# UnofficialJuliaMirrorSnapshots/TrajectoryOptimization.jl-c79d492b-0548-5874-b488-5a62c1d9d0ca

Hardware: AMD Instinct MI355X
Metric: iLQR iterations/sec (batched trajectories), quadrotor n=13 m=4 N=101 (higher is better)
Workload: dtype f64

## Files before the change

### trajectoryoptimization.jl-c79d492b-0548-5874-b488-5a62c1d9d0ca_amd/csrc/tog_bwd_team.hpp

```cpp
#pragma once
#include <type_traits>

namespace tog {

#define TEAM_FENCE() asm volatile("" ::: "memory")

constexpr int PX = 20;

template <class M>
struct TeamCfg {
  static constexpr int n = M::n, m = M::m, L = n + m;
  static constexpr int TEAM = (n + 1 <= 8) ? 8 : 16;
  static constexpr int TPW = WAVE / TEAM;
  static constexpr int cmax(int a, int b) { return a > b ? a : b; }
  static constexpr int PU = 2 * m;
  static constexpr int BUS =
      cmax(cmax(n * L, 3 * n * m), cmax(cmax(32 + n * m + n, n * n + n), cmax(m * m + n * m, n + PX + 2)));
  static constexpr int R2 = cmax(L * n, n * n + n);
  static constexpr int BUSP = cmax(BUS, n * L + R2);
  static constexpr int R2S = cmax(3 * m * m, m * m + 1);
  static constexpr int BUSPS = cmax(BUS, n * L + R2S);
  static constexpr int RQ = cmax(2 * n, n + PX);
};

// ... 13 lines not shown
__host__ __device__ inline int bwd_team_stride(int , int sqrt) {
  using C = TeamCfg<M>;
  int s = sqrt ? C::BUSPS : C::BUSP;
  s += sreg_size<M>(sqrt != 0);
  s += (34 - s % 32) % 32;
  return s;
}
inline size_t bwd_team_shmem(int stride, int tpw, int , int N) {
  return sizeof(double) * (size_t)stride * tpw + sizeof(int) * 2 * (size_t)N;
}

template <class M>
__host__ __device__ constexpr int ne_of() {
  return M::n + M::m + M::m * M::m + M::n * M::n;
}
constexpr int QPK = 4;
template <bool SQRT, bool AL>
__device__ __forceinline__ bool knot_dense(int k, int N, int cnt, int nx) {
  return k == N - 1 || (AL && (SQRT ? nx > 0 : cnt > 0));
}
template <class M>
__host__ __device__ inline int expand_team_stride(int pmax) {
  int s = 48 + pmax * 8 + pmax + M::n + M::m;
  return s + (s & 1);
}

constexpr int TEAM_MAX_ROWS = 128;
constexpr int TEAM_MAX_KNOTS = 1024;
inline bool team_rows_fit(const int* knot_off, const int* knot_cnt, const ConRow* rows, int N, int n, int m,
                          int nrows) {
  if (n + 1 > 16 || m > n || nrows > TEAM_MAX_ROWS || N > TEAM_MAX_KNOTS) return false;
  for (int k = 0; k < N; k++) {
    int nx = 0, nu = 0;
    if (knot_cnt[k] > PCAP) return false;
    for (int r = 0; r < knot_cnt[k]; r++) {
      const int t = rows[knot_off[k] + r].type;
      if (t == ROW_USER_INEQ || t == ROW_USER_EQ) return false;
      if (t == ROW_UMAX || t == ROW_UMIN) nu++;
      else nx++;
    }
    if (nx > PX || nu > 2 * m) return false;
  }
  return true;
}

template <class M, bool PT>
__device__ __forceinline__ void team_rows(const DevProblem* P, const DevBuffers& Bf, long long b, int k, int N, int pmax, int p,
                                          const ConRow* cr, const double* x, const double* u, RowInfo* rows,
                                          int* xr, int* ur, int& nx, int& nu, int team, int tl, int TEAM) {
  constexpr int n = M::n;
  const double* lam = Bf.lam + ((size_t)b * N + k) * pmax;
  const double* mu = Bf.mu + ((size_t)b * N + k) * pmax;
  const unsigned long long tmask = (TEAM >= 64 ? ~0ull : ((1ull << TEAM) - 1ull)) << (team * TEAM);
  const unsigned long long below = tmask & ((1ull << threadIdx.x) - 1ull);
  int cx = 0, cu = 0;
  for (int base = 0; base < p; base += TEAM) {
    const int r = base + tl;
    bool isx = false, isu = false;
    if (r < p) {
      const ConRow row = traj_row<PT>(P, b, cr[r]);
      const double c = row_value<false>(row, x, u);
      const double l = lam[r];
      const bool a = row_inequality<false>(row) ? ((c >= 0.0) || (l > 0.0)) : true;
      RowInfo ri;
      ri.w = a ? mu[r] : 0.0;
      ri.ws = a ? sqrt(mu[r]) : 0.0;
      ri.g = ri.w * c + l;
      ri.nnz = row_grad<false>(row, x, n, ri.idx, ri.v);
      rows[r] = ri;
      isu = (row.type == ROW_UMAX || row.type == ROW_UMIN);
      isx = !isu;
    }
    const unsigned long long bx = __ballot(isx) & tmask, bu = __ballot(isu) & tmask;
    if (isx) xr[cx + __popcll(bx & below)] = r;
    if (isu) ur[cu + __popcll(bu & below)] = r;
    cx += __popcll(bx);
    cu += __popcll(bu);
  }
  nx = cx;
  nu = cu;
}

__device__ __forceinline__ double row_at(const RowInfo& r, int col) {
  double v = 0.0;
  for (int z = 0; z < r.nnz; z++)
    if (r.idx[z] == col) v = r.v[z];
  return v;
}

template <class T>
__device__ __forceinline__ T opaque(T v) {
  asm volatile("" : "+v"(v));
  return v;
}

template <int L>
__device__ __forceinline__ double row_bcast(double v) {
  return __builtin_amdgcn_update_dpp(__builtin_nondeterministic_value(v), v, 0x150 + L, 0xF, 0xF, true);
}

template <int L>
__device__ __forceinline__ double quad_bcast(double v) {
  const long long x = __builtin_bit_cast(long long, v);
  const int lo = __builtin_amdgcn_update_dpp(__builtin_nondeterministic_value(0), (int)(x & 0xffffffffll), L * 0x55,
                                             0xF, 0xF, true);
  const int hi = __builtin_amdgcn_update_dpp(__builtin_nondeterministic_value(0), (int)(x >> 32), L * 0x55, 0xF, 0xF,
                                             true);
// ... 374 lines not shown
          team_qr<m + PU, m, m, TEAM, true>(a, m + PU, tl, bus);
        else
          team_qr<m + PU, m, m, TEAM>(a, m + nu, tl, bus);
#pragma unroll
        for (int i = 0; i < m; i++) Quuc[i] = (i <= tl) ? a[i] : 0.0;
      }
    }
    {
      double tx = 0.0;
      for (int z = 0; z < nx; z++) {
        const RowInfo& ri = rows[xr[z]];
        const double v = colx ? row_at(ri, c) : 0.0;
        if (v != 0.0) tx = fma(v, ri.g, tx);
      }
      Qxs += tx;
      if (!TERM) {
        double tu[m];
#pragma unroll
        for (int i = 0; i < m; i++) tu[i] = 0.0;
        for (int z = 0; z < nu; z++) {
          const RowInfo& ri = rows[ur[z]];
          const int id = ri.idx[0];
#pragma unroll
          for (int i = 0; i < m; i++)
            if (id == n + i) tu[i] = fma(ri.v[0], ri.g, tu[i]);
        }
#pragma unroll
        for (int i = 0; i < m; i++) Qu[i] += tu[i];
      }
    }
  }
  double* e = Bf.E + ((size_t)b * N + k) * NE;
  if (colx) e[tl] = Qxs;
  if (!TERM) {
    if (colu) {
      double qu = Qu[0];
#pragma unroll
      for (int i = 1; i < m; i++)
        if (tl == i) qu = Qu[i];
      e[n + tl] = qu;
#pragma unroll
      for (int i = 0; i < m; i++) e[n + m + i + m * tl] = Quuc[i];
    }
  }
  int nxk = 0;
  if (AL && SQRT) nxk = P->knot_nx[k];
  if (colx && knot_dense<SQRT, AL>(k, N, p, nxk)) {
#pragma unroll
    for (int i = 0; i < n; i++) e[n + m + m * m + i + n * tl] = Qxc[i];
  }
}

template <class M, int SQRTI, int ALI>
__global__ void __launch_bounds__(64) k_expand_team(const DevProblem* P, DevBuffers Bf, int mode) {
  using Cfg = TeamCfg<M>;
  extern __shared__ double expand_lds[];
  const int team = threadIdx.x / Cfg::TEAM, tl = threadIdx.x % Cfg::TEAM;
  const int N = P->N;
  const long long idx = (long long)blockIdx.x * Cfg::TPW + team;
  const long long slot = (mode == 2) ? idx : idx / N;
  const int k = (mode == 2) ? N - 1 : (int)(idx - slot * N);
  const long long b = traj_of_slot(Bf, slot, P->B);
  if (b < 0) return;
  if (!Bf.st[b].active || Bf.st[b].ls_pend) return;
  if (mode == 1 && k < N - 1 && !((ALI & 1) && P->knot_nx[k] > 0)) return;
  double* tlds = expand_lds + (size_t)team * expand_team_stride<M>(P->pmax);
  if (k == N - 1)
    team_expand<M, SQRTI != 0, (ALI & 1) != 0, true, (ALI & 2) != 0>(P, Bf, b, k, tlds, tl, team);
  else
    team_expand<M, SQRTI != 0, (ALI & 1) != 0, false, (ALI & 2) != 0>(P, Bf, b, k, tlds, tl, team);
}

template <class M, bool AL, bool PT>
__device__ __forceinline__ void quad_expand(const DevProblem* P, const DevBuffers& Bf, long long b, int k, int tl) {
  using Cfg = TeamCfg<M>;
  constexpr int n = M::n, m = M::m, PU = Cfg::PU, NE = ne_of<M>(), TQ = 4;
  static_assert(m <= TQ, "quad_expand: at most 4 controls");
  const int N = P->N, pmax = P->pmax;
  const double dt = P->dt;
  const bool colu = tl < m;
  const int cu = colu ? tl : 0;
  const double* xg = Bf.X + ((size_t)b * N + k) * n;
  const double* ug = Bf.U + ((size_t)b * (N - 1) + k) * m;
  constexpr int NXL = (n + TQ - 1) / TQ;
  double Qxs[NXL], Quuc[m], Qu[m];
  const int diag_mode = P->diag_cost;
  const CostView C_ = cost_at<n, m, PT>(P, k, b);
  if (diag_mode == 2) {
#pragma unroll
    for (int j = 0; j < NXL; j++) {
      const int cc = tl + TQ * j < n ? tl + TQ * j : 0;
      Qxs[j] = ((fma(C_.Q[cc + n * cc], xg[cc], 0.0) + C_.q[cc]) + 0.0) * dt;
    }
#pragma unroll
    for (int i = 0; i < m; i++) Qu[i] = ((fma(C_.R[i + m * i], ug[i], 0.0) + C_.r[i]) + 0.0) * dt;
    const double rd = C_.cR[cu + m * cu];
#pragma unroll
    for (int i = 0; i < m; i++) Quuc[i] = (i == cu) ? rd : 0.0;
  } else {
#pragma unroll
    for (int j = 0; j < NXL; j++) {
      const int cc = tl + TQ * j < n ? tl + TQ * j : 0;
      double a = 0.0, bq = 0.0;
      if (diag_mode) {
        a = fma(C_.Q[cc + n * cc], xg[cc], 0.0);
      } else {
#pragma unroll
        for (int jj = 0; jj < n; jj++) a = fma(C_.Q[cc + n * jj], xg[jj], a);
#pragma unroll
        for (int jj = 0; jj < m; jj++) bq = fma(C_.H[jj + m * cc], ug[jj], bq);
      }
      Qxs[j] = ((a + C_.q[cc]) + bq) * dt;
    }
#pragma unroll
    for (int i = 0; i < m; i++) {
      double a2 = 0.0, b2 = 0.0;
      if (diag_mode) {
        a2 = fma(C_.R[i + m * i], ug[i], 0.0);
      } else {
#pragma unroll
        for (int j = 0; j < m; j++) a2 = fma(C_.R[i + m * j], ug[j], a2);
#pragma unroll
        for (int j = 0; j < n; j++) b2 = fma(C_.H[i + m * j], xg[j], b2);
// ... 39 lines not shown
      return __builtin_amdgcn_update_dpp(__builtin_nondeterministic_value(0), rid[i / TQ], (i % TQ) * 0x55, 0xF, 0xF,
                                         true);
    };
    {
      double a[m + PU];
#pragma unroll
      for (int i = 0; i < m; i++) a[i] = Quuc[i];
      static_for<0, PU>([&](auto ic) {
        constexpr int i = decltype(ic)::value;
        const double ws = quad_bcast<i % TQ>(rws[i / TQ]), v = quad_bcast<i % TQ>(rv[i / TQ]);
        const int id = idx_of(ic);
        a[m + i] = (i < nu) ? ws * ((id == n + cu) ? v : 0.0) : 0.0;
      });
      team_qr<m + PU, m, m, TQ, true>(a, m + PU, tl, nullptr);
#pragma unroll
      for (int i = 0; i < m; i++) Quuc[i] = (i <= tl) ? a[i] : 0.0;
    }
    double tu[m];
#pragma unroll
    for (int i = 0; i < m; i++) tu[i] = 0.0;
    static_for<0, PU>([&](auto zc) {
      constexpr int z = decltype(zc)::value;
      const double v = quad_bcast<z % TQ>(rv[z / TQ]), g = quad_bcast<z % TQ>(rg[z / TQ]);
      const int id = idx_of(zc);
      if (z < nu) {
#pragma unroll
        for (int i = 0; i < m; i++)
          if (id == n + i) tu[i] = fma(v, g, tu[i]);
      }
    });
#pragma unroll
    for (int i = 0; i < m; i++) Qu[i] += tu[i];
    {
#pragma unroll
      for (int j = 0; j < NXL; j++) Qxs[j] += 0.0;
    }
  }
  double* e = Bf.E + ((size_t)b * N + k) * NE;
#pragma unroll
  for (int j = 0; j < NXL; j++)
    if (tl + TQ * j < n) e[tl + TQ * j] = Qxs[j];
  if (colu) {
    double qu = Qu[0];
#pragma unroll
    for (int i = 1; i < m; i++)
      if (tl == i) qu = Qu[i];
    e[n + tl] = qu;
#pragma unroll
    for (int i = 0; i < m; i++) e[n + m + i + m * tl] = Quuc[i];
  }
}

template <class M, int ALI>
__global__ void __launch_bounds__(64) __attribute__((amdgpu_waves_per_eu(5))) k_expand_u(const DevProblem* P, DevBuffers Bf) {
  const int team = threadIdx.x / 4, tl = threadIdx.x % 4;
  const int N = P->N;
  const long long idx = (long long)blockIdx.x * 16 + team;
  const long long slot = idx / (N - 1);
  const int k = (int)(idx - slot * (N - 1));
  const long long b = traj_of_slot(Bf, slot, P->B);
  if (b < 0) return;
  if (!Bf.st[b].active || Bf.st[b].ls_pend) return;
  if ((ALI & 1) && P->knot_nx[k] > 0) return;
  quad_expand<M, (ALI & 1) != 0, (ALI & 2) != 0>(P, Bf, b, k, tl);
}

#ifndef TOG_BWD_WAVES
#define TOG_BWD_WAVES 2
#endif
#ifndef TOG_TAIL_PF
#define TOG_TAIL_PF 0
#endif
#ifndef TOG_TAIL_TRI
#define TOG_TAIL_TRI 1
#endif
template <class M, int SQRTI, int ALI, int WPE>
__global__ void __launch_bounds__(64) __attribute__((amdgpu_waves_per_eu(WPE))) k_bwd_team(const DevProblem* P, DevBuffers Bf, int flags) {
  using Cfg = TeamCfg<M>;
  constexpr bool SQRT = SQRTI != 0, AL = (ALI & 1) != 0, TV = (ALI & 2) != 0;
  constexpr int n = M::n, m = M::m, L = n + m, TEAM = Cfg::TEAM, NQ = nq_of<M>(), NE = ne_of<M>();
  static_assert(m <= n && n + 1 <= TEAM, "team layout");
  extern __shared__ double team_lds[];
  const int team = threadIdx.x / TEAM, tl = threadIdx.x % TEAM;
  const long long bs = traj_of_slot(Bf, (long long)blockIdx.x * Cfg::TPW + team, P->B);
  const long long b = bs < 0 ? 0 : bs;
  const int N = P->N;
  const int stride = Bf.bwd_stride;
  constexpr int SREG = sreg_size<M>(SQRT);
  constexpr int SOFF = n * n;
  double* Sreg = team_lds + (size_t)team * stride;
  double* QU = Sreg + SOFF + n;
  double* bus = Sreg + SREG;
  int* kcnt = reinterpret_cast<int*>(team_lds + (size_t)Cfg::TPW * stride);
  int* knx = kcnt + N;
  if (AL) {
    for (int e = threadIdx.x; e < N; e += 64) {
      kcnt[e] = P->knot_cnt[e];
      knx[e] = P->knot_nx[e];
    }
    __syncthreads();
  }
  const bool live = bs >= 0 && Bf.st[b].active && !Bf.st[b].ls_pend;
  const bool store_S = (flags & TOG_BP_STORE_S) && Bf.Sdbg;
  const bool state_reg = (P->o.bp_reg_type == 1);
  const double dt = P->dt;
  const long long bb = live ? b : 0;
#define ABg (Bf.AB + (size_t)opaque(bb) * (N - 1) * n * L)
#define Kg (Bf.K + (size_t)opaque(bb) * (N - 1) * m * n)
#define dg (Bf.d + (size_t)opaque(bb) * (N - 1) * m)
#define Qs (Bf.Qscr + (size_t)opaque(bb) * N * NQ)
#define Eg (Bf.E + (size_t)opaque(bb) * N * NE)
  const bool colx = tl < n;
  const bool colu = tl < m;
  const int c = colx ? tl : 0;
  const int cu = colu ? tl : 0;
  auto lane_at = [&](double* base, int mul) { return base + opaque(tl) * mul; };
  RegState s;
// ... 901 lines not shown
```

### trajectoryoptimization.jl-c79d492b-0548-5874-b488-5a62c1d9d0ca_amd/csrc/tog_host_plan.hpp

```cpp
#pragma once
#include <algorithm>
#include <cmath>
#include <cstddef>
#include <cstring>
#include <type_traits>
#include <vector>

namespace tog_plan {

template <int... Vs, class F>
inline void pick(int v, F&& f) {
  (void)((v == Vs && (f(std::integral_constant<int, Vs>{}), true)) || ...);
}

enum TailBackward { TAIL_BWD_TEAM = 0, TAIL_BWD_QUAD = 1 };
constexpr long long TAIL_QUAD_ROUNDS = 1;
inline TailBackward tail_backward(long long width, int cus) {
  return (cus > 0 && width <= TAIL_QUAD_ROUNDS * (long long)cus) ? TAIL_BWD_QUAD : TAIL_BWD_TEAM;
}

constexpr int SPEC_WAVE = 64;
constexpr int SPEC_TAIL_PMAX = 16;
constexpr int SPEC_RQ = 4;
constexpr int SPEC_LANES = 32;
constexpr int SPEC_LDS_MAX = 64 * 1024;
constexpr int spec_tail_tc(int n, int m) { return (m * n <= 64) ? 16 : 8; }
constexpr int spec_tail_rec(int n, int m, int pmax) { return m * n + 2 * m + n + 2 * pmax; }
constexpr int spec_tail2_ring_off(int n, int m, int pmax) {
  return 2 * (spec_tail_tc(n, m) * spec_tail_rec(n, m, pmax) + 2 * pmax);
}
constexpr int spec_tail2_doubles(int n, int m, int pmax) {
  return spec_tail2_ring_off(n, m, pmax) + 2 * SPEC_RQ * (n + m) * SPEC_LANES +
         (SPEC_LANES * (int)sizeof(int) + (int)sizeof(double) - 1) / (int)sizeof(double) + SPEC_LANES;
}
inline int spec_tail2_lds(int n, int m, int pmax) {
  const size_t b = sizeof(double) * (size_t)spec_tail2_doubles(n, m, pmax);
  return (pmax <= SPEC_TAIL_PMAX && b <= (size_t)SPEC_LDS_MAX) ? (int)b : 0;
}
inline int spec_tail_lds(int n, int m, int pmax) {
  return pmax <= SPEC_TAIL_PMAX ? (int)(sizeof(double) * (spec_tail_tc(n, m) * spec_tail_rec(n, m, pmax) + 2 * pmax)) : 0;
}
inline bool spec_inline_diag(int cost_diag, int tv) { return cost_diag && !(tv & 2); }
constexpr bool spec_bulk_w1(int mn) { return mn > 64; }
enum SpecKernel { SPEC_TAIL3 = 0, SPEC_TAIL1 = 1, SPEC_BULK = 2, SPEC_BULK_W1 = 3 };
inline SpecKernel spec_kernel(int tail, int cand, int cost_diag, int tv, bool listed, int cnt, int tail2_lds,
                              int tail_lds, int mn) {
  const bool staged = tail && cand && spec_inline_diag(cost_diag, tv) && !listed;
  if (staged && tail2_lds > 0 && cnt <= SPEC_LANES) return SPEC_TAIL3;
  if (staged && tail_lds > 0 && cnt <= SPEC_WAVE) return SPEC_TAIL1;
  return spec_bulk_w1(mn) ? SPEC_BULK_W1 : SPEC_BULK;
}

inline bool chol_upper(const double* A, int n, double* U) {
  for (int i = 0; i < n * n; i++) U[i] = 0.0;
  for (int j = 0; j < n; j++) {
    double s = A[j + n * j];
    for (int k = 0; k < j; k++) s -= U[k + n * j] * U[k + n * j];
    if (!(s > 0.0)) return false;
    const double ujj = std::sqrt(s);
    U[j + n * j] = ujj;
    for (int c = j + 1; c < n; c++) {
      double t = A[j + n * c];
      for (int k = 0; k < j; k++) t -= U[k + n * j] * U[k + n * c];
      U[j + n * c] = t / ujj;
    }
  }
  return true;
}

struct CostPlan {
  int nc_in = 0, kst = 0, nk = 0;
// ... 106 lines not shown
```

### trajectoryoptimization.jl-c79d492b-0548-5874-b488-5a62c1d9d0ca_amd/csrc/tog_kernels.hpp

```cpp
#pragma once

#include "tog_device.hpp"
#include "tog_host_plan.hpp"
#include <string.h>

namespace tog {

constexpr int PCAP = 72;
template <class M>
__host__ __device__ constexpr int pcap_of() { return PCAP; }
constexpr int WAVE = 64;

__device__ __forceinline__ long long traj_of_slot(const DevBuffers& Bf, long long i, long long B) {
  if (Bf.act_list) return i < (long long)*Bf.act_count ? (long long)Bf.act_list[i] : -1;
  return i < B ? i : -1;
}
__device__ __forceinline__ long long slot_count(const DevBuffers& Bf, long long B) {
  return Bf.act_list ? (long long)*Bf.act_count : B;
}

__device__ __forceinline__ void wsync() { __syncthreads(); }

template <class M>
__host__ __device__ constexpr int cand_w() {
// ... 446 lines not shown
  s.zero_cnt = 0;
  s.grad = INFINITY;
  if (Bf.hist_in) {
    if (al) hist_outer(Bf, b, s, 0, s.J, s.c_max, s.mu_max);
    hist_inner(Bf, b, s, s.J, INFINITY, traj_gradient<M>(P, Bf, b, al));
  }
  Bf.st[b] = s;
}

template <class M, int INTEG>
__global__ void __launch_bounds__(64) k_rollout_open(const DevProblem* __restrict__ P, DevBuffers Bf) {
  const long long b = (long long)blockIdx.x * blockDim.x + threadIdx.x;
  if (b >= P->B) return;
  traj_rollout_open<M, INTEG>(P, Bf, b);
}

template <class M>
__global__ void __launch_bounds__(64) k_cost(const DevProblem* __restrict__ P, DevBuffers Bf, int al, int use_bar,
                                             double* Jout) {
  const long long b = (long long)blockIdx.x * blockDim.x + threadIdx.x;
  if (b >= P->B) return;
  constexpr int n = M::n, m = M::m;
  const int N = P->N;
  const double* X = (use_bar ? Bf.Xb : Bf.X) + (size_t)b * N * n;
  const double* U = (use_bar ? Bf.Ub : Bf.U) + (size_t)b * (N - 1) * m;
  Jout[b] = traj_cost<M>(P, Bf, b, X, U, al != 0, al ? Bf.C + (size_t)b * N * P->pmax : nullptr);
}

template <class M>
__global__ void __launch_bounds__(64) k_update_constraints(const DevProblem* __restrict__ P, DevBuffers Bf) {
  const long long b = (long long)blockIdx.x * blockDim.x + threadIdx.x;
  if (b >= P->B) return;
  constexpr int n = M::n, m = M::m;
  const int N = P->N, pmax = P->pmax;
  const double* X = Bf.X + (size_t)b * N * n;
  const double* U = Bf.U + (size_t)b * (N - 1) * m;
  for (int k = 0; k < N; k++) {
    const int cnt = knot_count(P, k);
    const cptr<ConRow> rows = knot_rows(P, k);
    for (int i = 0; i < cnt; i++)
      Bf.C[((size_t)b * N + k) * pmax + i] =
          row_value_m<M>(traj_row(P, b, uniform_row(load_row(rows + i))), X + (size_t)k * n, k < N - 1 ? U + (size_t)k * m : nullptr);
  }
}

template <class M, int INTEG>
__global__ void __launch_bounds__(64) k_rollout(const DevProblem* __restrict__ P, DevBuffers Bf, double alpha,
                                                int* ok) {
  const long long b = (long long)blockIdx.x * blockDim.x + threadIdx.x;
  if (b >= P->B) return;
  ok[b] = traj_rollout<M, INTEG>(P, Bf, b, alpha) ? 1 : 0;
}

template <class M, int INTEG, int W>
#ifndef TOG_JAC_WAVES
#define TOG_JAC_WAVES 1
#endif
__global__ void __launch_bounds__(256) __attribute__((amdgpu_waves_per_eu(TOG_JAC_WAVES)))
k_jacobian(const DevProblem* __restrict__ P, DevBuffers Bf, long long total) {
  using Mb = typename ModelTraits<M>::Base;
  constexpr int n = M::n, m = M::m, L = n + m, mb = Mb::m, Lb = n + mb, NCH = (Lb + W - 1) / W;
  const long long t = (long long)blockIdx.x * blockDim.x + threadIdx.x;
  if (t >= total) return;
  const int N = P->N;
  const int c = (int)(t % NCH);
  const long long bk = t / NCH;
  const int k = (int)(bk % (N - 1));
  const long long b = traj_of_slot(Bf, bk / (N - 1), P->B);
  if (b < 0 || !Bf.st[b].active || Bf.st[b].ls_pend) return;
  const double* x = Bf.X + ((size_t)b * N + k) * n;
  const double* u = Bf.U + ((size_t)b * (N - 1) + k) * m;
  Dual<W> xd[n], ud[mb], xn[n];
#pragma unroll
  for (int i = 0; i < n; i++) {
    xd[i].v = x[i];
#pragma unroll
    for (int w = 0; w < W; w++) xd[i].g[w] = (i == c * W + w) ? 1.0 : 0.0;
  }
#pragma unroll
  for (int i = 0; i < mb; i++) {
    ud[i].v = u[i];
#pragma unroll
    for (int w = 0; w < W; w++) ud[i].g[w] = (n + i == c * W + w) ? 1.0 : 0.0;
  }
  discrete_step<Mb, INTEG>(xn, xd, ud, P->dt);
  double* out = Bf.AB + ((size_t)b * (N - 1) + k) * n * L;
#pragma unroll
  for (int w = 0; w < W; w++) {
    const int col = c * W + w;
    if (col < Lb) {
#pragma unroll
      for (int i = 0; i < n; i++) out[i + n * col] = xn[i].g[w];
    }
  }
  if constexpr (ModelTraits<M>::slack > 0) {
    for (int j = c; j < n; j += NCH)
#pragma unroll
      for (int i = 0; i < n; i++) out[i + n * (Lb + j)] = (i == j) ? 1.0 : 0.0;
  }
}

template <class M, int INTEG, int W>
__global__ void __launch_bounds__(256) __attribute__((amdgpu_waves_per_eu(TOG_JAC_WAVES)))
k_jacobian_mt(const DevProblem* __restrict__ P, DevBuffers Bf, long long total) {
  using Mb = typename ModelTraits<M>::Core;
  constexpr int n = M::n, m = M::m, L = n + m, nb = Mb::n, mb = Mb::m, Lz = nb + mb + 1, NCH = (Lz + W - 1) / W;
  constexpr int SL = ModelTraits<M>::slack;
  const long long t = (long long)blockIdx.x * blockDim.x + threadIdx.x;
  if (t >= total) return;
  const int N = P->N;
  const int c = (int)(t % NCH);
  const long long bk = t / NCH;
  const int k = (int)(bk % (N - 1));
  const long long b = traj_of_slot(Bf, bk / (N - 1), P->B);
  if (b < 0 || !Bf.st[b].active || Bf.st[b].ls_pend) return;
  const double* x = Bf.X + ((size_t)b * N + k) * n;
  const double* u = Bf.U + ((size_t)b * (N - 1) + k) * m;
  const double h = u[m - 1];
  Dual<W> xd[nb], ud[mb], xn[nb + 1], dtd;
#pragma unroll
  for (int i = 0; i < nb; i++) {
    xd[i].v = x[i];
#pragma unroll
    for (int w = 0; w < W; w++) xd[i].g[w] = (i == c * W + w) ? 1.0 : 0.0;
  }
#pragma unroll
  for (int i = 0; i < mb; i++) {
    ud[i].v = u[i];
#pragma unroll
    for (int w = 0; w < W; w++) ud[i].g[w] = (nb + i == c * W + w) ? 1.0 : 0.0;
  }
  dtd.v = h * h;
#pragma unroll
  for (int w = 0; w < W; w++) dtd.g[w] = (nb + mb == c * W + w) ? 1.0 : 0.0;
  discrete_step<Mb, INTEG, Dual<W>, Dual<W>>(xn, xd, ud, dtd);
  double* out = Bf.AB + ((size_t)b * (N - 1) + k) * n * L;
#pragma unroll
  for (int w = 0; w < W; w++) {
    const int col = c * W + w;
    if (col < nb) {
#pragma unroll
      for (int i = 0; i < nb; i++) out[i + n * col] = xn[i].g[w];
      out[nb + n * col] = 0.0;
    } else if (col < nb + mb) {
#pragma unroll
      for (int i = 0; i < nb; i++) out[i + n * (n + col - nb)] = xn[i].g[w];
      out[nb + n * (n + col - nb)] = 0.0;
    } else if (col == nb + mb) {
#pragma unroll
      for (int i = 0; i < nb; i++) out[i + n * (n + m - 1)] = xn[i].g[w] * (2.0 * h);
      out[nb + n * (n + m - 1)] = 1.0;
    }
// ... 2604 lines not shown
```

### trajectoryoptimization.jl-c79d492b-0548-5874-b488-5a62c1d9d0ca_amd/csrc/tog_launch.hpp

```cpp
#pragma once

#include "tog_kernels.hpp"
#include "tog_host_plan.hpp"

namespace tog {

using tog_plan::pick;

inline int ali_backward(int al, int tv) { return (al ? 1 : 0) | ((tv & 1) ? 2 : 0); }
inline int ali_expand(int al, int tv) { return (al ? 1 : 0) | ((tv & 2) ? 2 : 0); }

struct StreamPair {
  hipStream_t st2;
  hipEvent_t fork, join;
};

struct ModelOps {
  int n, m;
  int slack;
  int pcap;
  int has_con;
  int min_time;
  long long jws_per_lane;
  void (*slack_controls)(const DevProblem*, const DevBuffers&, long long B, int integ, hipStream_t);
  void (*cost_expansion)(const DevProblem*, const DevBuffers&, long long B, int N, int sqrt, int al, int* fail,
                         hipStream_t);
  void (*init)(const DevProblem*, const DevBuffers&, long long B, int integ, int mode, hipStream_t);
  void (*refill)(const DevProblem*, const DevBuffers&, int count, int N, int integ, int mode, const int* list,
                 const double* x0, const double* U, const double* X, hipStream_t);
  void (*rollout_open)(const DevProblem*, const DevBuffers&, long long B, int integ, hipStream_t);
  void (*jacobian)(const DevProblem*, const DevBuffers&, long long B, int N, int integ, hipStream_t);
  void (*backward)(const DevProblem*, const DevBuffers&, long long B, int sqrt, int al, int flags, int team,
                   hipStream_t);
  void (*expand)(const DevProblem*, const DevBuffers&, long long B, int N, int pmax, int sqrt, int al, hipStream_t);
  void (*forward)(const DevProblem*, const DevBuffers&, long long B, int integ, int mode, int bookkeeping,
                  const double* Jprev, double* Jout, hipStream_t, const StreamPair* sp);
  void (*cost)(const DevProblem*, const DevBuffers&, long long B, int al, int use_bar, double* J, hipStream_t);
  void (*rollout)(const DevProblem*, const DevBuffers&, long long B, int integ, double alpha, int* ok, hipStream_t);
  void (*update_constraints)(const DevProblem*, const DevBuffers&, long long B, hipStream_t);
  int (*pn)(const DevProblem*, const DevBuffers&, const PNBuffers&, long long B, int integ, int phase, hipStream_t);
  int (*pn_wide)(const DevProblem*, const DevBuffers&, const PNWideBuffers&, long long slots, int integ, int phase,
                 hipStream_t);
  bool implicit;
  int bwd_lds_bytes;
  int team_tpw;
  int (*team_stride)(int pmax, int sqrt);
};

template <class M>
struct ModelLaunch {
#ifndef TOG_JW
#define TOG_JW 4
#endif
  using Mb = typename ModelTraits<M>::Base;
  static constexpr int JW = (Mb::n + Mb::m) <= 6 ? (Mb::n + Mb::m + (ModelTraits<M>::min_time ? 1 : 0))
                                                 : (Mb::id == TOG_MODEL_KUKA ? 1 : TOG_JW);
  static unsigned grid(long long total, int blk) { return (unsigned)((total + blk - 1) / blk); }
  template <class F>
  static void with_integ(int integ, F&& f) {
    if constexpr (!ModelTraits<M>::explicit_ok) {
      if (integ == TOG_RK3_IMPLICIT)
        f(std::integral_constant<int, TOG_RK3_IMPLICIT>{});
      else
        f(std::integral_constant<int, TOG_MIDPOINT_IMPLICIT>{});
      return;
    }
    if (integ == TOG_RK4) {
      f(std::integral_constant<int, TOG_RK4>{});
    } else if (integ == TOG_MIDPOINT) {
      f(std::integral_constant<int, TOG_MIDPOINT>{});
    } else if (integ == TOG_RK3_IMPLICIT || integ == TOG_MIDPOINT_IMPLICIT) {
      if constexpr (ModelTraits<M>::implicit_ok) {
        if (integ == TOG_RK3_IMPLICIT)
          f(std::integral_constant<int, TOG_RK3_IMPLICIT>{});
        else
          f(std::integral_constant<int, TOG_MIDPOINT_IMPLICIT>{});
      }
    } else {
      f(std::integral_constant<int, TOG_RK3>{});
    }
  }
  static void init(const DevProblem* P, const DevBuffers& Bf, long long B, int integ, int mode, hipStream_t st) {
    with_integ(integ, [&](auto ic) {
      constexpr int I = decltype(ic)::value;
      hipLaunchKernelGGL((k_init<M, I>), dim3(grid(B, 64)), dim3(64), 0, st, P, Bf, mode);
    });
  }
// ... 33 lines not shown
      constexpr int NCH = (Mb::n + Mb::m + JW - 1) / JW;
      const long long total = B * (long long)(N - 1) * NCH;
      with_integ(integ, [&](auto ic) {
        constexpr int I = decltype(ic)::value;
        hipLaunchKernelGGL((k_jacobian<M, I, JW>), dim3(grid(total, 256)), dim3(256), 0, st, P, Bf, total);
      });
    }
  }
  static void backward(const DevProblem* P, const DevBuffers& Bf, long long B, int sq, int al, int flags, int team,
                       hipStream_t st) {
    if constexpr (M::m <= M::n && M::n + 1 <= 16 && !ModelTraits<M>::min_time) {
    if (team) {
      constexpr int TPW = TeamCfg<M>::TPW;
      const dim3 g((unsigned)((B + TPW - 1) / TPW)), blk(64);
      DevBuffers Bl = Bf;
      Bl.bwd_stride = Bf.bwd_stride2[sq ? 1 : 0];
      Bl.bwd_shmem = Bf.bwd_shmem2[sq ? 1 : 0];
      const unsigned sm = (unsigned)Bl.bwd_shmem;
      const int ali = ali_backward(al, Bf.tv);
      auto launch = [&](auto wpe_c) {
        pick<0, 1>(sq ? 1 : 0, [&](auto sq_c) {
          pick<0, 1, 2, 3>(ali, [&](auto ali_c) {
            hipLaunchKernelGGL((k_bwd_team<M, decltype(sq_c)::value, decltype(ali_c)::value, decltype(wpe_c)::value>),
                               g, blk, sm, st, P, Bl, flags);
          });
        });
      };
      const char* tk = getenv("TOG_BWD_TAIL");
      const bool quad = (tk && !strcmp(tk, "team"))   ? false
                        : (tk && !strcmp(tk, "quad")) ? true
                                                      : tog_plan::tail_backward(B, Bf.simds / 4) == tog_plan::TAIL_BWD_QUAD;
      if (Bf.tail && sq && TeamCfg<M>::TEAM == 16 && quad) {
        if constexpr (TeamCfg<M>::TEAM == 16) {
          pick<0, 1, 2, 3>(ali, [&](auto ali_c) {
            hipLaunchKernelGGL((k_bwd_quad<M, decltype(ali_c)::value>), dim3((unsigned)B), dim3(256), 0, st, P, Bf,
                               flags);
          });
        }
      } else if (Bf.tail || (B + TPW - 1) / TPW <= Bf.simds) {
        launch(std::integral_constant<int, 1>{});
      } else {
        launch(std::integral_constant<int, TOG_BWD_WAVES>{});
      }
      return;
    }
    }
    pick<0, 1>(sq ? 1 : 0, [&](auto sq_c) {
      pick<0, 1>(al ? 1 : 0, [&](auto al_c) {
        hipLaunchKernelGGL((k_backward<M, decltype(sq_c)::value, decltype(al_c)::value>), dim3((unsigned)B), dim3(64),
                           0, st, P, Bf, flags);
      });
    });
  }
  static void expand(const DevProblem* P, const DevBuffers& Bf, long long B, int N, int pmax, int sq, int al,
                     hipStream_t st) {
    if constexpr (M::m <= M::n && M::n + 1 <= 16 && !ModelTraits<M>::min_time) {
      constexpr int TPW = TeamCfg<M>::TPW;
      const unsigned sm = (unsigned)(sizeof(double) * TPW * expand_team_stride<M>(pmax));
      int mode = 0;
      const int ali = ali_expand(al, Bf.tv);
      if constexpr (M::m <= 4 && TeamCfg<M>::TEAM == 16) {
        const char* eq = getenv("TOG_EXPAND_QUAD");
        if (sq && !(eq && eq[0] == '0')) {
          const long long qteams = B * (long long)(N - 1);
          pick<0, 1, 2, 3>(ali, [&](auto ali_c) {
            hipLaunchKernelGGL((k_expand_u<M, decltype(ali_c)::value>), dim3((unsigned)((qteams + 15) / 16)), dim3(64),
                               0, st, P, Bf);
          });
          mode = (al && Bf.dense_stage_knots) ? 1 : 2;
        }
      }
      const long long teams = (mode == 2) ? B : B * (long long)N;
      const dim3 g((unsigned)((teams + TPW - 1) / TPW)), blk(64);
      pick<0, 1>(sq ? 1 : 0, [&](auto sq_c) {
        pick<0, 1, 2, 3>(ali, [&](auto ali_c) {
          hipLaunchKernelGGL((k_expand_team<M, decltype(sq_c)::value, decltype(ali_c)::value>), g, blk, sm, st, P, Bf,
                             mode);
        });
      });
    }
  }
  template <int INTEG>
  static void spec(const DevProblem* P, const DevBuffers& Bf, long long B, int mode, int lo, int cnt, const int* list,
                   const int* count, hipStream_t st) {
    const bool diag = tog_plan::spec_inline_diag(Bf.cost_diag, Bf.tv);
    const tog_plan::SpecKernel kern =
        tog_plan::spec_kernel(Bf.tail, Bf.cand ? 1 : 0, Bf.cost_diag, Bf.tv, list != nullptr, cnt,
                              Bf.spec_tail2_shmem, Bf.spec_tail_shmem, M::n * M::m);
    if (kern == tog_plan::SPEC_TAIL3) {
      hipLaunchKernelGGL((k_ls_spec_tail2<M, INTEG, 1>), dim3((unsigned)B), dim3(3 * WAVE),
                         (unsigned)Bf.spec_tail2_shmem, st, P, Bf, mode, lo, cnt);
      return;
    }
    if (kern == tog_plan::SPEC_TAIL1) {
      hipLaunchKernelGGL((k_ls_spec_tail<M, INTEG, 1>), dim3((unsigned)B), dim3(WAVE), (unsigned)Bf.spec_tail_shmem, st,
                         P, Bf, mode, lo, cnt);
      return;
    }
    const unsigned gs = grid(B * (long long)cnt, 256);
    const unsigned rb = (mode == TOG_MODE_AL) ? (unsigned)Bf.rows_lds : 0u;
    pick<0, 1>(Bf.cand ? 1 : 0, [&](auto cand_c) {
      pick<0, 1>(rb ? 1 : 0, [&](auto lrt_c) {
        pick<0, 1>(diag ? 1 : 0, [&](auto diag_c) {
          constexpr bool CAND = decltype(cand_c)::value != 0, LRT = decltype(lrt_c)::value != 0;
          constexpr int DC = CAND ? decltype(diag_c)::value : 0;
          if constexpr (tog_plan::spec_bulk_w1(M::n * M::m))
            hipLaunchKernelGGL((k_ls_spec_w1<M, INTEG, CAND, LRT, DC>), dim3(grid(B * (long long)cnt, 64)), dim3(64),
                               LRT ? rb : 0u, st, P, Bf, mode, lo, cnt, list, count);
          else
            hipLaunchKernelGGL((k_ls_spec<M, INTEG, CAND, LRT, DC>), dim3(gs), dim3(256), LRT ? rb : 0u, st, P, Bf,
                               mode, lo, cnt, list, count);
        });
      });
    });
  }
  template <int INTEG>
  static void forward_cand(const DevProblem* P, const DevBuffers& Bf, long long B, int mode, int bk, const double* Jp,
                           double* Jo, hipStream_t st) {
    const int F = Bf.ls_first;
    const unsigned knots_lds = (unsigned)(Bf.nknots * (2 * sizeof(double) + sizeof(int)));
    if (F >= Bf.nc && bk && Bf.tail) {
      const char* lf = getenv("TOG_LS_FINISH");
      if (!(lf && !strcmp(lf, "split"))) {
        spec<INTEG>(P, Bf, B, mode, 0, Bf.nc, nullptr, nullptr, st);
        const unsigned rows = (mode == TOG_MODE_AL) ? (unsigned)Bf.rows_lds : 0u;
        hipLaunchKernelGGL((k_ls_finish<M, INTEG>), dim3((unsigned)B), dim3(LS_FINISH_THREADS),
                           knots_lds > rows ? knots_lds : rows, st, P, Bf, mode, Jp, Jo);
        return;
      }
    }
    (void)hipMemsetAsync(Bf.ls_count, 0, sizeof(int) * LS_COUNT_SLOTS, st);
    if (F >= Bf.nc) {
      spec<INTEG>(P, Bf, B, mode, 0, Bf.nc, nullptr, nullptr, st);
// ... 113 lines not shown
        rc = hipFuncSetAttribute(reinterpret_cast<const void*>(kern), hipFuncAttributeMaxDynamicSharedMemorySize, (int)lds);
        if (rc != hipSuccess) return;
      }
      hipLaunchKernelGGL(kern, dim3((unsigned)B), dim3(T), lds, st, P, Bf, W);
    };
    if (phase == 0)
      hipLaunchKernelGGL((k_pn_begin<M, INTEG, T>), dim3((unsigned)B), dim3(T), 0, st, P, Bf, W);
    else if (phase == 1)
      big(k_pn_project<M, INTEG, T>);
    else if (phase == 2)
      hipLaunchKernelGGL((k_pn_finish<M, INTEG, T>), dim3((unsigned)B), dim3(T), 0, st, P, Bf, W);
    else {
      if (phase == 3)
        big(k_pn_kkt<M, INTEG, T>);
      else if (phase == 4)
        big(k_pn_ls_begin<M, INTEG, T>);
      else if (phase == 5)
        big(k_pn_ls_proj<M, INTEG, T>);
      else
        big(k_pn_ls_end<M, INTEG, T>);
    }
    return rc;
  }
  static int pn(const DevProblem* P, const DevBuffers& Bf, const PNBuffers& W, long long B, int integ, int phase,
                hipStream_t st) {
    hipError_t rc = hipSuccess;
    with_integ(integ, [&](auto ic) { rc = pn_phase<decltype(ic)::value, WAVE>(P, Bf, W, B, phase, st); });
    return (int)rc;
  }
  static int pn_wide(const DevProblem* P, const DevBuffers& Bf, const PNWideBuffers& W, long long slots, int integ,
                     int phase, hipStream_t st) {
    hipError_t rc = hipSuccess;
    with_integ(integ, [&](auto ic) { rc = pn_phase<decltype(ic)::value, PN_WIDE_THREADS>(P, Bf, W, slots, phase, st); });
    return (int)rc;
  }
  static ModelOps ops() {
    ModelOps o;
    o.n = M::n;
    o.m = M::m;
    o.slack = ModelTraits<M>::slack;
    o.pcap = pcap_of<M>();
    o.has_con = HasCon<M>::value ? 1 : 0;
    o.min_time = ModelTraits<M>::min_time ? 1 : 0;
    o.jws_per_lane = (Mb::id == TOG_MODEL_KUKA && !ModelTraits<M>::min_time) ? 2LL * M::n * 2 : 0;
    o.implicit = ModelTraits<M>::implicit_ok;
    o.slack_controls = slack_controls;
    o.cost_expansion = cost_expansion;
    o.init = init;
    o.refill = refill;
    o.rollout_open = rollout_open;
    o.jacobian = jacobian;
    o.backward = backward;
    o.expand = expand;
    o.forward = forward;
    o.cost = cost;
    o.rollout = rollout;
    o.update_constraints = update_constraints;
    if constexpr (M::n + M::m <= PN_SM_MAX) {
      o.pn = pn;
      o.pn_wide = pn_wide;
    } else {
      o.pn = nullptr;
      o.pn_wide = nullptr;
    }
    o.bwd_lds_bytes = (int)sizeof(BwdLds<M, true>);
    o.team_tpw = TeamCfg<M>::TPW;
    o.team_stride = bwd_team_stride<M>;
    return o;
  }
};

}
```

### trajectoryoptimization.jl-c79d492b-0548-5874-b488-5a62c1d9d0ca_amd/csrc/tog_runtime.cpp

```cpp
#include <cmath>
#include <hip/hip_runtime.h>
#include <math.h>
#include <string.h>

#include <string>
#include <chrono>
#include <thread>
#include <vector>

#include <dlfcn.h>

#include "tog_plugin.hpp"
#include "tog_host_plan.hpp"
#include "tog_traj_tables.hpp"
#include "tog_stream.hpp"
#include "tog_cost_plugin.hpp"

using namespace tog;

#define TOG_BUILTIN_MODELS(X)                        \
  X(TOG_MODEL_DOUBLE_INTEGRATOR, double_integrator)  \
  X(TOG_MODEL_CARTPOLE, cartpole)                    \
  X(TOG_MODEL_QUADROTOR, quadrotor)                  \
  X(TOG_MODEL_CAR, car)                              \
// ... 1649 lines not shown
int32_t tog_rollout(tog_handle* h, double alpha, int32_t* ok_out) {
  if (!h) return fail(TOG_ERR_ARG, "null handle");
  if (is_multi(h))
    return each_part(h, [&](tog_handle* p, size_t o) { return tog_rollout(p, alpha, ok_out ? ok_out + o : nullptr); });
  HIPCHECK(hipSetDevice(h->device));
  h->ops->rollout(h->dP, h->buf, h->B, h->integ, alpha, h->d_iscratch, h->stream);
  HIPCHECK(hipGetLastError());
  if (ok_out) {
    HIPCHECK(hipMemcpyAsync(ok_out, h->d_iscratch, sizeof(int) * h->B, hipMemcpyDeviceToHost, h->stream));
    HIPCHECK(hipStreamSynchronize(h->stream));
  }
  return TOG_OK;
}

int32_t tog_solve_init(tog_handle* h, int32_t mode) {
  if (!h) return fail(TOG_ERR_ARG, "null handle");
  if (is_multi(h)) {
    h->mode = mode;
    return each_part(h, [&](tog_handle* p, size_t) { return tog_solve_init(p, mode); });
  }
  if (mode != TOG_MODE_ILQR && mode != TOG_MODE_AL) return fail(TOG_ERR_ARG, "mode");
  HIPCHECK(hipSetDevice(h->device));
  h->mode = mode;
  h->last_active = -1.0;
  h->stats_pending = false;
  h->ops->init(h->dP, h->buf, h->B, h->integ, mode, h->stream);
  if (h->d_slot_job)
    hipLaunchKernelGGL(k_slot_iota, dim3((unsigned)((h->B + 255) / 256)), dim3(256), 0, h->stream, h->d_slot_job,
                       (long long)h->B);
  HIPCHECK(hipGetLastError());
  return TOG_OK;
}

int32_t tog_solve_step(tog_handle* h, int32_t nsteps) {
  if (!h) return fail(TOG_ERR_ARG, "null handle");
  if (is_multi(h)) return each_part(h, [&](tog_handle* p, size_t) { return tog_solve_step(p, nsteps); });
  HIPCHECK(hipSetDevice(h->device));
  const int al = (h->mode == TOG_MODE_AL);
  const double few = 65536.0 / h->buf.nc;
  h->buf.ls_first = ((double)h->B <= few || (h->last_active >= 0.0 && h->last_active <= few)) ? h->buf.nc : LS_FIRST;
  h->buf.tail = ((double)h->B <= TAIL_ACTIVE || (h->last_active >= 0.0 && h->last_active <= TAIL_ACTIVE)) ? 1 : 0;
  DevBuffers Bt = h->buf;
  long long Bl = h->B;
  if (h->buf.tail && h->last_active >= 0.0 && h->last_active < (double)h->B && !getenv("TOG_NO_COMPACT")) {
    if (h->last_active == 0.0) return TOG_OK;
    Bl = (long long)ceil(h->last_active);
    HIPCHECK(hipMemsetAsync(h->d_act_count, 0, sizeof(int), h->stream));
    hipLaunchKernelGGL(k_list_active, dim3((unsigned)((h->B + 255) / 256)), dim3(256), 0, h->stream, h->buf.st,
                       (long long)h->B, h->d_act_list, h->d_act_count);
    Bt.act_list = h->d_act_list;
    Bt.act_count = h->d_act_count;
  }
  for (int i = 0; i < nsteps; i++) {
    timed(h, TOG_KERNEL_JACOBIAN, [&] { h->ops->jacobian(h->dP, Bt, Bl, h->N, h->integ, h->stream); });
    if (h->bwd_team)
      timed(h, TOG_KERNEL_EXPANSION, [&] {
        h->ops->expand(h->dP, Bt, Bl, h->N, h->pmax, h->opts.square_root, al, h->stream);
      });
    timed(h, TOG_KERNEL_BACKWARD,
          [&] { h->ops->backward(h->dP, Bt, Bl, h->opts.square_root, al, 0, h->bwd_team, h->stream); });
    timed(h, TOG_KERNEL_FORWARD,
          [&] { h->ops->forward(h->dP, Bt, Bl, h->integ, h->mode, 1, nullptr, nullptr, h->stream, &h->sp); });
  }
  HIPCHECK(hipGetLastError());
  return TOG_OK;
}

int32_t tog_batch_stats_device(tog_handle* h, void* dptr3) {
  if (!h || !dptr3) return fail(TOG_ERR_ARG, "null argument");
  if (is_multi(h)) return fail(TOG_ERR_UNSUPPORTED, "device pointers are per device: use tog_batch_stats");
  HIPCHECK(hipSetDevice(h->device));
  hipLaunchKernelGGL(k_batch_stats, dim3(1), dim3(1024), 0, h->stream, h->buf.st, (long long)h->B, (double*)dptr3);
  HIPCHECK(hipGetLastError());
  return TOG_OK;
}

int32_t tog_batch_stats(tog_handle* h, double* out3) {
  if (!h || !out3) return fail(TOG_ERR_ARG, "null argument");
  int32_t rc = tog_batch_stats_begin(h);
  return rc ? rc : tog_batch_stats_end(h, out3);
}

int32_t tog_batch_stats_begin(tog_handle* h) {
  if (!h) return fail(TOG_ERR_ARG, "null handle");
  if (is_multi(h)) return each_part(h, [](tog_handle* p, size_t) { return tog_batch_stats_begin(p); });
  HIPCHECK(hipSetDevice(h->device));
  if (h->stats_pending) return fail(TOG_ERR_ARG, "tog_batch_stats_begin: the previous check was not ended");
  if (!h->h_stats) HIPCHECK(hipHostMalloc((void**)&h->h_stats, sizeof(double) * 4, hipHostMallocDefault));
  if (!h->stats_ev) HIPCHECK(hipEventCreateWithFlags(&h->stats_ev, hipEventDisableTiming));
  int rc = tog_batch_stats_device(h, h->d_stats);
  if (rc) return rc;
  HIPCHECK(hipMemcpyAsync(h->h_stats, h->d_stats, sizeof(double) * 3, hipMemcpyDeviceToHost, h->stream));
  HIPCHECK(hipEventRecord(h->stats_ev, h->stream));
  h->stats_pending = true;
  return TOG_OK;
}

int32_t tog_batch_stats_end(tog_handle* h, double* out3) {
  if (!h || !out3) return fail(TOG_ERR_ARG, "null argument");
  if (is_multi(h)) {
    double acc[3] = {0.0, 0.0, 0.0};
    for (tog_handle* p : h->parts) {
      double v[3];
      int32_t rc = tog_batch_stats_end(p, v);
      if (rc) return rc;
      acc[0] += v[0];
      acc[1] += v[1];
      acc[2] = tog_jlmax(acc[2], v[2]);
// ... 689 lines not shown
```

Measured before the change: 93940.

## Fuse tail-phase Jacobian and cost-expansion kernels into one role-split launch

Adds a k_tail_prepare kernel that partitions its blocks into Jacobian, quad-expansion and team-expansion roles, so the tail phase (few active trajectories) issues one launch instead of two or three. Jacobian and expand bodies are factored into device item functions, and a host planner sizes the block ranges and LDS. It targets launch overhead and serialization between small kernels when the batch is nearly converged. In exchange, the fused kernel has the heavier register and LDS footprint of all roles, and the ballot mask now uses the logical team lane instead of threadIdx.x.

Result: faster. 95430 (median of 6 runs) (+1.6%).

```diff
diff --git a/trajectoryoptimization.jl-c79d492b-0548-5874-b488-5a62c1d9d0ca_amd/csrc/tog_bwd_team.hpp b/trajectoryoptimization.jl-c79d492b-0548-5874-b488-5a62c1d9d0ca_amd/csrc/tog_bwd_team.hpp
--- a/trajectoryoptimization.jl-c79d492b-0548-5874-b488-5a62c1d9d0ca_amd/csrc/tog_bwd_team.hpp
+++ b/trajectoryoptimization.jl-c79d492b-0548-5874-b488-5a62c1d9d0ca_amd/csrc/tog_bwd_team.hpp
@@ -89,7 +89,7 @@
   const double* lam = Bf.lam + ((size_t)b * N + k) * pmax;
   const double* mu = Bf.mu + ((size_t)b * N + k) * pmax;
   const unsigned long long tmask = (TEAM >= 64 ? ~0ull : ((1ull << TEAM) - 1ull)) << (team * TEAM);
-  const unsigned long long below = tmask & ((1ull << threadIdx.x) - 1ull);
+  const unsigned long long below = tmask & ((1ull << (team * TEAM + tl)) - 1ull);
   int cx = 0, cu = 0;
   for (int base = 0; base < p; base += TEAM) {
     const int r = base + tl;
@@ -570,23 +570,28 @@
 }
 
 template <class M, int SQRTI, int ALI>
-__global__ void __launch_bounds__(64) k_expand_team(const DevProblem* P, DevBuffers Bf, int mode) {
-  using Cfg = TeamCfg<M>;
-  extern __shared__ double expand_lds[];
-  const int team = threadIdx.x / Cfg::TEAM, tl = threadIdx.x % Cfg::TEAM;
+__device__ __forceinline__ void expand_team_item(const DevProblem* P, const DevBuffers& Bf, int mode, long long idx,
+                                                 double* lds, int lteam, int wteam, int tl) {
   const int N = P->N;
-  const long long idx = (long long)blockIdx.x * Cfg::TPW + team;
   const long long slot = (mode == 2) ? idx : idx / N;
   const int k = (mode == 2) ? N - 1 : (int)(idx - slot * N);
   const long long b = traj_of_slot(Bf, slot, P->B);
   if (b < 0) return;
   if (!Bf.st[b].active || Bf.st[b].ls_pend) return;
   if (mode == 1 && k < N - 1 && !((ALI & 1) && P->knot_nx[k] > 0)) return;
-  double* tlds = expand_lds + (size_t)team * expand_team_stride<M>(P->pmax);
+  double* tlds = lds + (size_t)lteam * expand_team_stride<M>(P->pmax);
   if (k == N - 1)
-    team_expand<M, SQRTI != 0, (ALI & 1) != 0, true, (ALI & 2) != 0>(P, Bf, b, k, tlds, tl, team);
+    team_expand<M, SQRTI != 0, (ALI & 1) != 0, true, (ALI & 2) != 0>(P, Bf, b, k, tlds, tl, wteam);
   else
-    team_expand<M, SQRTI != 0, (ALI & 1) != 0, false, (ALI & 2) != 0>(P, Bf, b, k, tlds, tl, team);
+    team_expand<M, SQRTI != 0, (ALI & 1) != 0, false, (ALI & 2) != 0>(P, Bf, b, k, tlds, tl, wteam);
+}
+
+template <class M, int SQRTI, int ALI>
+__global__ void __launch_bounds__(64) k_expand_team(const DevProblem* P, DevBuffers Bf, int mode) {
+  using Cfg = TeamCfg<M>;
+  extern __shared__ double expand_lds[];
+  const int team = threadIdx.x / Cfg::TEAM, tl = threadIdx.x % Cfg::TEAM;
+  expand_team_item<M, SQRTI, ALI>(P, Bf, mode, (long long)blockIdx.x * Cfg::TPW + team, expand_lds, team, team, tl);
 }
 
 template <class M, bool AL, bool PT>
@@ -732,10 +737,8 @@
 }
 
 template <class M, int ALI>
-__global__ void __launch_bounds__(64) __attribute__((amdgpu_waves_per_eu(5))) k_expand_u(const DevProblem* P, DevBuffers Bf) {
-  const int team = threadIdx.x / 4, tl = threadIdx.x % 4;
+__device__ __forceinline__ void expand_quad_item(const DevProblem* P, const DevBuffers& Bf, long long idx, int tl) {
   const int N = P->N;
-  const long long idx = (long long)blockIdx.x * 16 + team;
   const long long slot = idx / (N - 1);
   const int k = (int)(idx - slot * (N - 1));
   const long long b = traj_of_slot(Bf, slot, P->B);
@@ -743,6 +746,34 @@
   if (!Bf.st[b].active || Bf.st[b].ls_pend) return;
   if ((ALI & 1) && P->knot_nx[k] > 0) return;
   quad_expand<M, (ALI & 1) != 0, (ALI & 2) != 0>(P, Bf, b, k, tl);
+}
+
+template <class M, int ALI>
+__global__ void __launch_bounds__(64) __attribute__((amdgpu_waves_per_eu(5))) k_expand_u(const DevProblem* P, DevBuffers Bf) {
+  const int team = threadIdx.x / 4, tl = threadIdx.x % 4;
+  expand_quad_item<M, ALI>(P, Bf, (long long)blockIdx.x * 16 + team, tl);
+}
+
+template <class M, int INTEG, int SQRTI, int ALI, int W>
+__global__ void __launch_bounds__(tog_plan::PREP_THREADS) __attribute__((amdgpu_waves_per_eu(TOG_JAC_WAVES)))
+k_tail_prepare(const DevProblem* __restrict__ P, DevBuffers Bf, long long jtotal, unsigned jac, unsigned quad,
+               int mode) {
+  using Cfg = TeamCfg<M>;
+  extern __shared__ double expand_lds[];
+  const int role = tog_plan::prepare_role(blockIdx.x, jac, quad);
+  const long long blk = (long long)tog_plan::prepare_block(blockIdx.x, jac, quad);
+  if (role == tog_plan::PREP_JAC) {
+    const long long t = blk * tog_plan::PREP_THREADS + threadIdx.x;
+    if (t >= jtotal) return;
+    jacobian_item<M, INTEG, W>(P, Bf, t);
+  } else if (role == tog_plan::PREP_QUAD) {
+    if constexpr (M::m <= 4 && Cfg::TEAM == 16)
+      expand_quad_item<M, ALI>(P, Bf, blk * tog_plan::PREP_QUADS + threadIdx.x / 4, threadIdx.x % 4);
+  } else {
+    const int lteam = threadIdx.x / Cfg::TEAM, tl = threadIdx.x % Cfg::TEAM;
+    expand_team_item<M, SQRTI, ALI>(P, Bf, mode, blk * (tog_plan::PREP_THREADS / Cfg::TEAM) + lteam, expand_lds, lteam,
+                                    lteam % Cfg::TPW, tl);
+  }
 }
 
 #ifndef TOG_BWD_WAVES
diff --git a/trajectoryoptimization.jl-c79d492b-0548-5874-b488-5a62c1d9d0ca_amd/csrc/tog_host_plan.hpp b/trajectoryoptimization.jl-c79d492b-0548-5874-b488-5a62c1d9d0ca_amd/csrc/tog_host_plan.hpp
--- a/trajectoryoptimization.jl-c79d492b-0548-5874-b488-5a62c1d9d0ca_amd/csrc/tog_host_plan.hpp
+++ b/trajectoryoptimization.jl-c79d492b-0548-5874-b488-5a62c1d9d0ca_amd/csrc/tog_host_plan.hpp
@@ -17,6 +17,40 @@
 constexpr long long TAIL_QUAD_ROUNDS = 1;
 inline TailBackward tail_backward(long long width, int cus) {
   return (cus > 0 && width <= TAIL_QUAD_ROUNDS * (long long)cus) ? TAIL_BWD_QUAD : TAIL_BWD_TEAM;
+}
+
+constexpr int PREP_THREADS = 256;
+constexpr int PREP_QUADS = PREP_THREADS / 4;
+enum PrepareRole { PREP_JAC = 0, PREP_QUAD = 1, PREP_TEAM = 2 };
+constexpr int prepare_role(unsigned blk, unsigned jac, unsigned quad) {
+  return blk < jac ? PREP_JAC : (blk - jac < quad ? PREP_QUAD : PREP_TEAM);
+}
+constexpr unsigned prepare_block(unsigned blk, unsigned jac, unsigned quad) {
+  return blk < jac ? blk : (blk - jac < quad ? blk - jac : blk - jac - quad);
+}
+struct TailPrepare {
+  bool fused = false;
+  unsigned jac = 0, quad = 0, team = 0;
+  unsigned lds = 0;
+  unsigned blocks() const { return jac + quad + team; }
+};
+inline TailPrepare tail_prepare(int tail, int bwd_team, bool plain_jac, bool split, long long width, int N, int nch,
+                                int team_lanes, int mode, int team_stride) {
+  TailPrepare p;
+  if (!tail || !bwd_team || !plain_jac || split || width <= 0 || N < 2) return p;
+  const long long tpb = PREP_THREADS / team_lanes;
+  const long long jt = width * (long long)(N - 1) * nch, qt = mode ? width * (long long)(N - 1) : 0;
+  const long long tt = mode == 2 ? width : width * (long long)N;
+  const long long jb = (jt + PREP_THREADS - 1) / PREP_THREADS, qb = (qt + PREP_QUADS - 1) / PREP_QUADS;
+  const long long tb = (tt + tpb - 1) / tpb;
+  const long long lds = (long long)sizeof(double) * tpb * team_stride;
+  if (lds > 64 * 1024 || jb + qb + tb > 0x7fffffffLL) return p;
+  p.fused = true;
+  p.jac = (unsigned)jb;
+  p.quad = (unsigned)qb;
+  p.team = (unsigned)tb;
+  p.lds = (unsigned)lds;
+  return p;
 }
 
 constexpr int SPEC_WAVE = 64;
diff --git a/trajectoryoptimization.jl-c79d492b-0548-5874-b488-5a62c1d9d0ca_amd/csrc/tog_kernels.hpp b/trajectoryoptimization.jl-c79d492b-0548-5874-b488-5a62c1d9d0ca_amd/csrc/tog_kernels.hpp
--- a/trajectoryoptimization.jl-c79d492b-0548-5874-b488-5a62c1d9d0ca_amd/csrc/tog_kernels.hpp
+++ b/trajectoryoptimization.jl-c79d492b-0548-5874-b488-5a62c1d9d0ca_amd/csrc/tog_kernels.hpp
@@ -522,16 +522,13 @@
   ok[b] = traj_rollout<M, INTEG>(P, Bf, b, alpha) ? 1 : 0;
 }
 
-template <class M, int INTEG, int W>
 #ifndef TOG_JAC_WAVES
 #define TOG_JAC_WAVES 1
 #endif
-__global__ void __launch_bounds__(256) __attribute__((amdgpu_waves_per_eu(TOG_JAC_WAVES)))
-k_jacobian(const DevProblem* __restrict__ P, DevBuffers Bf, long long total) {
+template <class M, int INTEG, int W>
+__device__ __forceinline__ void jacobian_item(const DevProblem* P, const DevBuffers& Bf, long long t) {
   using Mb = typename ModelTraits<M>::Base;
   constexpr int n = M::n, m = M::m, L = n + m, mb = Mb::m, Lb = n + mb, NCH = (Lb + W - 1) / W;
-  const long long t = (long long)blockIdx.x * blockDim.x + threadIdx.x;
-  if (t >= total) return;
   const int N = P->N;
   const int c = (int)(t % NCH);
   const long long bk = t / NCH;
@@ -568,6 +565,14 @@
 #pragma unroll
       for (int i = 0; i < n; i++) out[i + n * (Lb + j)] = (i == j) ? 1.0 : 0.0;
   }
+}
+
+template <class M, int INTEG, int W>
+__global__ void __launch_bounds__(256) __attribute__((amdgpu_waves_per_eu(TOG_JAC_WAVES)))
+k_jacobian(const DevProblem* __restrict__ P, DevBuffers Bf, long long total) {
+  const long long t = (long long)blockIdx.x * blockDim.x + threadIdx.x;
+  if (t >= total) return;
+  jacobian_item<M, INTEG, W>(P, Bf, t);
 }
 
 template <class M, int INTEG, int W>
diff --git a/trajectoryoptimization.jl-c79d492b-0548-5874-b488-5a62c1d9d0ca_amd/csrc/tog_launch.hpp b/trajectoryoptimization.jl-c79d492b-0548-5874-b488-5a62c1d9d0ca_amd/csrc/tog_launch.hpp
--- a/trajectoryoptimization.jl-c79d492b-0548-5874-b488-5a62c1d9d0ca_amd/csrc/tog_launch.hpp
+++ b/trajectoryoptimization.jl-c79d492b-0548-5874-b488-5a62c1d9d0ca_amd/csrc/tog_launch.hpp
@@ -33,6 +33,8 @@
   void (*backward)(const DevProblem*, const DevBuffers&, long long B, int sqrt, int al, int flags, int team,
                    hipStream_t);
   void (*expand)(const DevProblem*, const DevBuffers&, long long B, int N, int pmax, int sqrt, int al, hipStream_t);
+  int (*tail_prepare)(const DevProblem*, const DevBuffers&, long long B, int N, int pmax, int integ, int sqrt, int al,
+                      int team, hipStream_t);
   void (*forward)(const DevProblem*, const DevBuffers&, long long B, int integ, int mode, int bookkeeping,
                   const double* Jprev, double* Jout, hipStream_t, const StreamPair* sp);
   void (*cost)(const DevProblem*, const DevBuffers&, long long B, int al, int use_bar, double* J, hipStream_t);
@@ -172,22 +174,27 @@
       });
     });
   }
+  static int expand_mode(const DevBuffers& Bf, int sq, int al) {
+    if constexpr (M::m <= 4 && TeamCfg<M>::TEAM == 16) {
+      const char* eq = getenv("TOG_EXPAND_QUAD");
+      if (sq && !(eq && eq[0] == '0')) return (al && Bf.dense_stage_knots) ? 1 : 2;
+    }
+    return 0;
+  }
   static void expand(const DevProblem* P, const DevBuffers& Bf, long long B, int N, int pmax, int sq, int al,
                      hipStream_t st) {
     if constexpr (M::m <= M::n && M::n + 1 <= 16 && !ModelTraits<M>::min_time) {
       constexpr int TPW = TeamCfg<M>::TPW;
       const unsigned sm = (unsigned)(sizeof(double) * TPW * expand_team_stride<M>(pmax));
-      int mode = 0;
+      const int mode = expand_mode(Bf, sq, al);
       const int ali = ali_expand(al, Bf.tv);
       if constexpr (M::m <= 4 && TeamCfg<M>::TEAM == 16) {
-        const char* eq = getenv("TOG_EXPAND_QUAD");
-        if (sq && !(eq && eq[0] == '0')) {
+        if (mode) {
           const long long qteams = B * (long long)(N - 1);
           pick<0, 1, 2, 3>(ali, [&](auto ali_c) {
             hipLaunchKernelGGL((k_expand_u<M, decltype(ali_c)::value>), dim3((unsigned)((qteams + 15) / 16)), dim3(64),
                                0, st, P, Bf);
           });
-          mode = (al && Bf.dense_stage_knots) ? 1 : 2;
         }
       }
       const long long teams = (mode == 2) ? B : B * (long long)N;
@@ -199,6 +206,32 @@
         });
       });
     }
+  }
+  static int tail_prepare(const DevProblem* P, const DevBuffers& Bf, long long B, int N, int pmax, int integ, int sq,
+                          int al, int team, hipStream_t st) {
+    if constexpr (M::m <= M::n && M::n + 1 <= 16 && !ModelTraits<M>::min_time && Mb::id != TOG_MODEL_KUKA &&
+                  ModelTraits<M>::explicit_ok) {
+      constexpr int NCH = (Mb::n + Mb::m + JW - 1) / JW;
+      const bool plain = integ == TOG_RK3 || integ == TOG_RK4 || integ == TOG_MIDPOINT;
+      const char* tp = getenv("TOG_TAIL_PREPARE");
+      const int mode = expand_mode(Bf, sq, al);
+      const tog_plan::TailPrepare pl = tog_plan::tail_prepare(Bf.tail, team, plain, tp && !strcmp(tp, "split"), B, N, NCH,
+                                                              TeamCfg<M>::TEAM, mode, expand_team_stride<M>(pmax));
+      if (!pl.fused) return 0;
+      const long long jtotal = B * (long long)(N - 1) * NCH;
+      const int ali = ali_expand(al, Bf.tv);
+      pick<TOG_RK3, TOG_RK4, TOG_MIDPOINT>(integ, [&](auto ic) {
+        pick<0, 1>(sq ? 1 : 0, [&](auto sq_c) {
+          pick<0, 1, 2, 3>(ali, [&](auto ali_c) {
+            hipLaunchKernelGGL(
+                (k_tail_prepare<M, decltype(ic)::value, decltype(sq_c)::value, decltype(ali_c)::value, JW>),
+                dim3(pl.blocks()), dim3(tog_plan::PREP_THREADS), pl.lds, st, P, Bf, jtotal, pl.jac, pl.quad, mode);
+          });
+        });
+      });
+      return 1;
+    }
+    return 0;
   }
   template <int INTEG>
   static void spec(const DevProblem* P, const DevBuffers& Bf, long long B, int mode, int lo, int cnt, const int* list,
@@ -418,6 +451,7 @@
     o.jacobian = jacobian;
     o.backward = backward;
     o.expand = expand;
+    o.tail_prepare = tail_prepare;
     o.forward = forward;
     o.cost = cost;
     o.rollout = rollout;
diff --git a/trajectoryoptimization.jl-c79d492b-0548-5874-b488-5a62c1d9d0ca_amd/csrc/tog_runtime.cpp b/trajectoryoptimization.jl-c79d492b-0548-5874-b488-5a62c1d9d0ca_amd/csrc/tog_runtime.cpp
--- a/trajectoryoptimization.jl-c79d492b-0548-5874-b488-5a62c1d9d0ca_amd/csrc/tog_runtime.cpp
+++ b/trajectoryoptimization.jl-c79d492b-0548-5874-b488-5a62c1d9d0ca_amd/csrc/tog_runtime.cpp
@@ -1725,8 +1725,13 @@
     Bt.act_count = h->d_act_count;
   }
   for (int i = 0; i < nsteps; i++) {
-    timed(h, TOG_KERNEL_JACOBIAN, [&] { h->ops->jacobian(h->dP, Bt, Bl, h->N, h->integ, h->stream); });
-    if (h->bwd_team)
+    int fused = 0;
+    timed(h, TOG_KERNEL_JACOBIAN, [&] {
+      fused = h->ops->tail_prepare(h->dP, Bt, Bl, h->N, h->pmax, h->integ, h->opts.square_root, al, h->bwd_team,
+                                   h->stream);
+      if (!fused) h->ops->jacobian(h->dP, Bt, Bl, h->N, h->integ, h->stream);
+    });
+    if (h->bwd_team && !fused)
       timed(h, TOG_KERNEL_EXPANSION, [&] {
         h->ops->expand(h->dP, Bt, Bl, h->N, h->pmax, h->opts.square_root, al, h->stream);
       });
```
